# levia-than/neptune-pde-solver

Hardware: AMD Instinct MI355X
Metric: stencil-cell-updates/s (higher is better)
Workload: dtype f64

## Files before the change

### neptune-pde-solver_amd/csrc/kernels/apply_march2.hpp

```cpp
#pragma once
#include "apply_march.hpp"

namespace neptune_hip {

template <class T, int NIN>
struct March2Params {
  const T* in[NIN];
  T* out;
  int32_t N0, N1, N2;
  int32_t plb[3], pub[3];
  int64_t olb[3];
  int32_t rI0, rI1;
  int32_t chunk;
  uint32_t nJ, nK;
};

template <class T, class FP, int NS>
struct March2Geom {
  static constexpr int VK = 16 / (int)sizeof(T), G = 64 / (int)sizeof(T);
  static constexpr int R0 = FP::R0, R1 = FP::R1, R2 = FP::R2;
  static constexpr int HG = G / 2 > VK ? G / 2 : VK;
  static constexpr int MK = (NS * R2 + HG - 1) / HG * HG;
  static constexpr int SPAN = kWave * VK, KEEPK = SPAN - 2 * MK;
  static constexpr int MJ = NS * R1;
  static constexpr int WARM = 2 * R0 * (NS - 1);
};

template <class T, int NIN>
struct Leapfrog2Params : March2Params<T, NIN> {
  T* out_v;
};

template <class Body, class T, int NIN, class FP, int NS, int RJ, int WJ, int MINW, bool LF = false>
__global__ __launch_bounds__(kWave* WJ, MINW) void neptune_apply_march2(
    std::conditional_t<LF, Leapfrog2Params<T, NIN>, March2Params<T, NIN>> P, Body body) {
  using V = typename Vec16<T>::type;
  using GM = March2Geom<T, FP, NS>;
  constexpr int VK = GM::VK, R0 = GM::R0, R1 = GM::R1, R2 = GM::R2, NP = 2 * R0 + 1;
  static_assert(NS >= 2 && NS <= 3, "two or three applies per pass");
  static_assert(!LF || (NS == 2 && NIN >= 2), "leapfrog: two stages, input 1 = the previous state");
  constexpr int TJ = RJ * WJ;
  constexpr int MK = GM::MK, SPAN = GM::SPAN;
  static_assert(R0 >= 1 && R0 <= 2 && R1 >= 1 && R1 <= 2 && R2 >= 1 && R2 <= 2 && !FP::BOX && FP::HALO_MASK == 1u, "star of input 0, radius 1..2");
  static_assert(RJ >= R1 && R2 <= VK && TJ > 2 * GM::MJ, "window too small for the footprint");
  constexpr int NQ = (NS - 1) * R0 + 1;
  constexpr int NF = NIN > 1 ? NIN - 1 : 1;
  __shared__ V lds[2][WJ][NS][2 * R1][kWave];

  const int lane = threadIdx.x & (kWave - 1);
  const int w = __builtin_amdgcn_readfirstlane(threadIdx.x >> 6);
  const uint32_t vb = xcd_remap(blockIdx.x, gridDim.x);
  const uint32_t kt = vb % P.nK;
  const uint32_t t = vb / P.nK;
  const uint32_t jt = t % P.nJ;
  const uint32_t ct = t / P.nJ;

  const int32_t Jb = (int32_t)(jt * (TJ - 2 * GM::MJ)) - GM::MJ;
  const int32_t j0 = Jb + w * RJ;
  const int32_t kw = (int32_t)(kt * GM::KEEPK) - MK;
  const int32_t k0 = kw + lane * VK;
  const int32_t kc = k0 < 0 ? 0 : (k0 > P.N2 - VK ? P.N2 - VK : k0);
  const uint32_t lane_b = (uint32_t)kc * (uint32_t)sizeof(T);
  uint32_t rowb[RJ];
  static_for<RJ>([&](auto rc) {
    constexpr int r = rc;
    int32_t j = j0 + r;
    j = j < 0 ? 0 : (j >= P.N1 ? P.N1 - 1 : j);
    rowb[r] = (uint32_t)j * (uint32_t)P.N2 * (uint32_t)sizeof(T);
  });
  const int64_t plane_b = (int64_t)P.N1 * P.N2 * (int64_t)sizeof(T);

  const int32_t ib = P.rI0 + (int32_t)ct * P.chunk;
  const int32_t ie = (ib + P.chunk < P.rI1) ? ib + P.chunk : P.rI1;
  if (ib >= ie) return;

  auto load_plane = [&](const T* field, int32_t ip, V(&rows)[RJ]) {
    const int32_t ic = ip < 0 ? 0 : (ip >= P.N0 ? P.N0 - 1 : ip);
    const char* base = reinterpret_cast<const char*>(field) + (int64_t)ic * plane_b;
    static_for<RJ>([&](auto rc) {
      constexpr int r = rc;
      rows[r] = *reinterpret_cast<const V*>(base + (rowb[r] + lane_b));
    });
  };

  bool row_keep[RJ], in_j[RJ], in_k[VK];
  static_for<RJ>([&](auto rc) {
    constexpr int r = rc;
    const int32_t j = j0 + r;
    row_keep[r] = j >= Jb + GM::MJ && j < Jb + TJ - GM::MJ && j >= 0 && j < P.N1;
    in_j[r] = j >= P.plb[1] && j < P.pub[1];
  });
  static_for<VK>([&](auto ec) {
    constexpr int e = ec;
    in_k[e] = (k0 + e) >= P.plb[2] && (k0 + e) < P.pub[2];
  });
  const bool lane_keep = k0 >= kw + MK && k0 < kw + SPAN - MK && k0 >= 0 && k0 < P.N2;

  auto stage = [&](const V(&pl)[NP][RJ], const V(&above)[R1], const V(&below)[R1], const V(&fx)[NF][NQ][RJ], const V(&xp)[RJ],
                   auto qc, int32_t ip, V(&res)[RJ]) {
    constexpr int q = decltype(qc)::value;
    V ring[1][NP][RJ + 2 * R1];
    T lft[1][1][RJ + 2 * R1][R2], rgt[1][1][RJ + 2 * R1][R2];
    V pt[NIN][RJ];
    static_for<RJ>([&](auto rc) {
      constexpr int r = rc;
      static_for<NP>([&](auto pc) { constexpr int pp = pc; ring[0][pp][r + R1] = pl[pp][r]; });
      static_for<R2>([&](auto xc) {
        constexpr int x = xc;
        constexpr int dl = R2 - x, dr = x + 1;
        lft[0][0][r + R1][x] = from_prev<true>(pl[R0][r][VK - dl], pl[R0][r][0], lane);
        rgt[0][0][r + R1][x] = from_next<true>(pl[R0][r][dr - 1], pl[R0][r][VK - 1], lane);
      });
      static_for<NIN>([&](auto nc) {
        constexpr int n = nc;
        if constexpr (LF && n == 1) pt[n][r] = xp[r];
        else if constexpr (n > 0) pt[n][r] = fx[n - 1][q][r];
      });
    });
    static_for<R1>([&](auto xc) {
      constexpr int x = xc;
      ring[0][R0][x] = above[x];
      ring[0][R0][RJ + R1 + x] = below[x];
    });
    const bool in_i = ip >= P.plb[0] && ip < P.pub[0];
    const int64_t li = (int64_t)ip + P.olb[0];
    static_for<RJ>([&](auto rc) {
      constexpr int r = rc;
      const int64_t lj = (int64_t)(j0 + r) + P.olb[1];
      static_for<VK>([&](auto ec) {
        constexpr int e = ec;
        const int64_t lk = (int64_t)(k0 + e) + P.olb[2];
        MarchAcc<T, 3, NIN, FP, RJ, r, e, false> acc{ring, lft, rgt, pt, li, lj, lk};
        const T val = body(acc);
        const T through = pl[R0][r][e];
        res[r][e] = (in_i && in_j[r] && in_k[e]) ? val : OutsideOf<Body, T>::apply(body, through);
      });
    });
  };

  V ring[NS][NP][RJ];
  V un[RJ];
  V fx[NF][NQ][RJ], fn[NF][RJ];
  V wres[RJ];
  const int32_t i0 = ib - GM::WARM;
  static_for<NP - 1>([&](auto pc) { constexpr int pp = pc; load_plane(P.in[0], i0 + NS * R0 - 2 * R0 + pp, ring[0][pp]); });
  load_plane(P.in[0], i0 + NS * R0, un);
  if constexpr (NIN > 1) {
    static_for<NIN - 1>([&](auto nc) {
      constexpr int n = nc;
      if constexpr (!(LF && n == 0))
        static_for<NQ - 1>([&](auto qc) { constexpr int q = qc; load_plane(P.in[n + 1], i0 + q, fx[n][q]); });
      load_plane(P.in[n + 1], i0 + NQ - 1, fn[n]);
    });
  }
  static_for<NS - 1>([&](auto kc) {
    constexpr int k = kc + 1;
    static_for<NP - 1>([&](auto pc) { constexpr int pp = pc; static_for<RJ>([&](auto rc) { constexpr int r = rc; ring[k][pp][r] = ring[0][0][r]; }); });
  });

  for (int32_t i = i0; i < ie; ++i) {
    static_for<RJ>([&](auto rc) { constexpr int r = rc; ring[0][NP - 1][r] = un[r]; });
    if constexpr (NIN > 1)
      static_for<NIN - 1>([&](auto nc) { constexpr int n = nc; static_for<RJ>([&](auto rc) { constexpr int r = rc; fx[n][NQ - 1][r] = fn[n][r]; }); });
    const int buf = (i - i0) & 1;
    static_for<NS>([&](auto kc) {
      constexpr int k = kc;
      static_for<R1>([&](auto xc) {
        constexpr int x = xc;
        lds[buf][w][k][x][lane] = ring[k][R0][x];
        lds[buf][w][k][R1 + x][lane] = ring[k][R0][RJ - R1 + x];
      });
    });
    __syncthreads();
    V above[NS][R1], below[NS][R1];
    static_for<NS>([&](auto kc) {
      constexpr int k = kc;
      static_for<R1>([&](auto xc) {
        constexpr int x = xc;
        above[k][x] = ring[k][R0][0];
        below[k][x] = ring[k][R0][RJ - 1];
        if (w > 0) above[k][x] = lds[buf][w - 1][k][R1 + x][lane];
        if (w < WJ - 1) below[k][x] = lds[buf][w + 1][k][x][lane];
      });
    });
    if (i + NS * R0 + 1 <= ie - 1 + NS * R0) {
      load_plane(P.in[0], i + NS * R0 + 1, un);
      if constexpr (NIN > 1) static_for<NIN - 1>([&](auto nc) { constexpr int n = nc; load_plane(P.in[n + 1], i + NQ, fn[n]); });
    }
    static_for<NS>([&](auto kc) {
      constexpr int k = kc;
      constexpr int q = (NS - k - 1) * R0;
      const V(&xp)[RJ] = (LF && k == 0) ? fx[0][NQ - 1] : ring[0][0];
      if constexpr (k + 1 < NS) stage(ring[k], above[k], below[k], fx, xp, std::integral_constant<int, q>{}, i + q, ring[k + 1][NP - 1]);
      else stage(ring[k], above[k], below[k], fx, xp, std::integral_constant<int, 0>{}, i, wres);
    });
    if (i >= ib && lane_keep) {
      char* obase = reinterpret_cast<char*>(P.out) + (int64_t)i * plane_b;
      static_for<RJ>([&](auto rc) {
        constexpr int r = rc;
        if (row_keep[r]) __builtin_nontemporal_store(wres[r], reinterpret_cast<V*>(obase + (rowb[r] + lane_b)));
      });
    }
    if constexpr (LF) {
      if (i + R0 >= ib && i + R0 < ie && lane_keep) {
        char* obase = reinterpret_cast<char*>(P.out_v) + (int64_t)(i + R0) * plane_b;
        static_for<RJ>([&](auto rc) {
          constexpr int r = rc;
          if (row_keep[r]) __builtin_nontemporal_store(ring[1][NP - 1][r], reinterpret_cast<V*>(obase + (rowb[r] + lane_b)));
        });
      }
    }
    static_for<NS>([&](auto kc) {
      constexpr int k = kc;
      static_for<NP - 1>([&](auto pc) { constexpr int pp = pc; static_for<RJ>([&](auto rc) { constexpr int r = rc; ring[k][pp][r] = ring[k][pp + 1][r]; }); });
    });
    if constexpr (NIN > 1)
      static_for<NIN - 1>([&](auto nc) {
        constexpr int n = nc;
        if constexpr (!(LF && n == 0))
          static_for<NQ - 1>([&](auto qc) { constexpr int q = qc; static_for<RJ>([&](auto rc) { constexpr int r = rc; fx[n][q][r] = fx[n][q + 1][r]; }); });
      });
  }
}


struct March2R2Params {
  const void* in[NEPTUNE_HIP_MAX_INPUTS];
  void* out;
  int32_t N0, N1;
  int32_t plb[2], pub[2];
  int64_t olb[2];
  int32_t rI0, rI1;
  int32_t chunk;
  uint32_t nK;
};

template <class FP>
constexpr bool march2_rank2_footprint() {
  return FP::MARCH_OK && !FP::BOX && FP::HALO_MASK == 1u && FP::R0 >= 1 && FP::R0 <= 2 && FP::R1 == 0 && FP::R2 >= 1 && FP::R2 <= 2;
}

struct Leapfrog2R2Params : March2R2Params {
  void* out_v;
};

template <class Body, class T, int NIN, class FP, int NS, int PF, bool LF = false>
__global__ __launch_bounds__(256) void neptune_apply_march2_rank2(std::conditional_t<LF, Leapfrog2R2Params, March2R2Params> P, Body body) {
  using V = typename Vec16<T>::type;
  using GM = March2Geom<T, FP, NS>;
  constexpr int VK = GM::VK, R0 = GM::R0, R2 = GM::R2, NP = 2 * R0 + 1, MK = GM::MK, SPAN = GM::SPAN, KEEPK = GM::KEEPK;
  static_assert(NS >= 2 && NS <= 3 && march2_rank2_footprint<FP>() && R2 <= VK, "window constants");
  static_assert(!LF || (NS == 2 && NIN >= 2), "leapfrog: two stages, input 1 = the previous state");
  constexpr int NQ = (NS - 1) * R0 + 1;
  constexpr int NF = NIN > 1 ? NIN - 1 : 1;
  const int lane = threadIdx.x & (kWave - 1);
  const uint32_t gw = blockIdx.x * (blockDim.x / kWave) + (threadIdx.x >> 6);
  const uint32_t kt = gw % P.nK, ct = gw / P.nK;
  const int32_t kw = (int32_t)(kt * KEEPK) - MK;
  const int32_t k0 = kw + lane * VK;
  const int32_t kc = k0 < 0 ? 0 : (k0 > P.N1 - VK ? P.N1 - VK : k0);
  const int32_t ib = P.rI0 + (int32_t)ct * P.chunk;
  const int32_t ie = (ib + P.chunk < P.rI1) ? ib + P.chunk : P.rI1;
  if (ib >= ie) return;
  T* out = static_cast<T*>(P.out);
  auto load_row = [&](int n, int32_t ip) -> V {
    const int32_t ic = ip < 0 ? 0 : (ip >= P.N0 ? P.N0 - 1 : ip);
    return *reinterpret_cast<const V*>(static_cast<const T*>(P.in[n]) + (int64_t)ic * P.N1 + kc);
  };
  bool in_k[VK];
  static_for<VK>([&](auto ec) { constexpr int e = ec; in_k[e] = (k0 + e) >= P.plb[1] && (k0 + e) < P.pub[1]; });
  const bool lane_keep = k0 >= kw + MK && k0 < kw + SPAN - MK && k0 >= 0 && k0 < P.N1;

  auto stage = [&](const V(&pl)[NP], const V(&fx)[NF][NQ], const V& xp, auto qc, int32_t ip) -> V {
    constexpr int q = decltype(qc)::value;
    V ring[1][NP][1];
    T lft[1][1][1][R2], rgt[1][1][1][R2];
    V pt[NIN][1];
    static_for<NP>([&](auto pc) { constexpr int pp = pc; ring[0][pp][0] = pl[pp]; });
    static_for<R2>([&](auto xc) {
      constexpr int x = xc;
      constexpr int dl = R2 - x, dr = x + 1;
      lft[0][0][0][x] = from_prev<true>(pl[R0][VK - dl], pl[R0][0], lane);
      rgt[0][0][0][x] = from_next<true>(pl[R0][dr - 1], pl[R0][VK - 1], lane);
    });
    static_for<NIN>([&](auto nc) {
      constexpr int n = nc;
      if constexpr (LF && n == 1) pt[n][0] = xp;
      else if constexpr (n > 0) pt[n][0] = fx[n - 1][q];
    });
    const bool in_i = ip >= P.plb[0] && ip < P.pub[0];
    const int64_t li = (int64_t)ip + P.olb[0];
    V res;
    static_for<VK>([&](auto ec) {
      constexpr int e = ec;
      const int64_t lk = (int64_t)(k0 + e) + P.olb[1];
      MarchAcc<T, 2, NIN, FP, 1, 0, e, false> acc{ring, lft, rgt, pt, li, 0, lk};
      const T val = body(acc);
      res[e] = (in_i && in_k[e]) ? val : OutsideOf<Body, T>::apply(body, pl[R0][e]);
    });
    return res;
  };

  V ring[NS][NP];
  V un[PF];
  V fx[NF][NQ], fn[NF][PF];
  const int32_t i0 = ib - GM::WARM;
  static_for<NP - 1>([&](auto pc) { constexpr int pp = pc; ring[0][pp] = load_row(0, i0 + NS * R0 - 2 * R0 + pp); });
  static_for<PF>([&](auto dc) { constexpr int d = dc; un[d] = load_row(0, i0 + NS * R0 + d); });
  if constexpr (NIN > 1) {
    static_for<NIN - 1>([&](auto nc) {
      constexpr int n = nc;
      if constexpr (!(LF && n == 0)) static_for<NQ - 1>([&](auto qc) { constexpr int q = qc; fx[n][q] = load_row(n + 1, i0 + q); });
      static_for<PF>([&](auto dc) { constexpr int d = dc; fn[n][d] = load_row(n + 1, i0 + NQ - 1 + d); });
    });
  }
  static_for<NS - 1>([&](auto kc2) { constexpr int k = kc2 + 1; static_for<NP - 1>([&](auto pc) { constexpr int pp = pc; ring[k][pp] = ring[0][0]; }); });
  auto step = [&](int32_t i, auto slot_c) {
    constexpr int slot = slot_c;
    ring[0][NP - 1] = un[slot];
    if constexpr (NIN > 1) static_for<NIN - 1>([&](auto nc) { constexpr int n = nc; fx[n][NQ - 1] = fn[n][slot]; });
    if (i + NS * R0 + PF <= ie - 1 + NS * R0) {
      un[slot] = load_row(0, i + NS * R0 + PF);
      if constexpr (NIN > 1) static_for<NIN - 1>([&](auto nc) { constexpr int n = nc; fn[n][slot] = load_row(n + 1, i + NQ - 1 + PF); });
    }
    V w;
    static_for<NS>([&](auto kc2) {
      constexpr int k = kc2;
      constexpr int q = (NS - k - 1) * R0;
      const V& xp = (LF && k == 0) ? fx[0][NQ - 1] : ring[0][0];
      if constexpr (k + 1 < NS) ring[k + 1][NP - 1] = stage(ring[k], fx, xp, std::integral_constant<int, q>{}, i + q);
      else w = stage(ring[k], fx, xp, std::integral_constant<int, 0>{}, i);
    });
    if (i >= ib && lane_keep) __builtin_nontemporal_store(w, reinterpret_cast<V*>(out + (int64_t)i * P.N1 + kc));
    if constexpr (LF) {
      if (i + R0 >= ib && i + R0 < ie && lane_keep)
        __builtin_nontemporal_store(ring[1][NP - 1], reinterpret_cast<V*>(static_cast<T*>(P.out_v) + (int64_t)(i + R0) * P.N1 + kc));
    }
    static_for<NS>([&](auto kc2) { constexpr int k = kc2; static_for<NP - 1>([&](auto pc) { constexpr int pp = pc; ring[k][pp] = ring[k][pp + 1]; }); });
    if constexpr (NIN > 1)
      static_for<NIN - 1>([&](auto nc) {
        constexpr int n = nc;
        if constexpr (!(LF && n == 0)) static_for<NQ - 1>([&](auto qc) { constexpr int q = qc; fx[n][q] = fx[n][q + 1]; });
      });
  };
  for (int32_t i = i0; i < ie; i += PF) {
    static_for<PF>([&](auto phc) {
      constexpr int ph = phc;
      if (i + ph < ie) step(i + ph, phc);
    });
  }
}


template <class T, int NIN, class FP>
inline bool march2_rank2_eligible(const neptune_hip_apply_geom_t* g, const void* const* in, const void* out) {
  constexpr int G = 64 / (int)sizeof(T);
  if (!g || g->rank != 2 || g->num_inputs != NIN) return false;
  if (!march2_rank2_footprint<FP>()) return false;
  int64_t n[2];
  const int r[2] = {FP::R0, FP::R2};
  for (int d = 0; d < 2; ++d) {
    n[d] = g->out_ub[d] - g->out_lb[d];
    for (int k = 0; k < NIN; ++k)
      if (g->in_lb[k][d] != g->out_lb[d] || g->in_ub[k][d] != g->out_ub[d]) return false;
    if (g->lb[d] < g->ub[d] && (g->lb[d] - r[d] < g->out_lb[d] || g->ub[d] + r[d] > g->out_ub[d])) return false;
  }
  if (g->region_lb[1] != 0 || g->region_ub[1] != n[1]) return false;
  if (n[1] % G != 0 || n[1] < 2 * G || n[0] < 1 || n[0] >= 0x7fffffffLL || n[1] >= 0x7fffffffLL) return false;
  if ((uintptr_t)out % 64 != 0) return false;
  for (int k = 0; k < NIN; ++k)
    if (!in[k] || (uintptr_t)in[k] % 64 != 0) return false;
  return true;
}

template <class Body, class T, int NIN, class FP, int NS, bool LF = false>
inline int launch_march2_rank2(const Body& body, const neptune_hip_apply_geom_t* g, const void* const* in, void* out, hipStream_t stream,
                               int chunk_req, void* out_v = nullptr) {
  if (!march2_rank2_eligible<T, NIN, FP>(g, in, out) || geom_bounds_empty(g)) return NEPTUNE_HIP_EUNSUPPORTED;
  constexpr int KEEPK = March2Geom<T, FP, NS>::KEEPK, PF = 4;
  std::conditional_t<LF, Leapfrog2R2Params, March2R2Params> P{};
  if constexpr (LF) P.out_v = out_v;
  for (int k = 0; k < NIN; ++k) P.in[k] = in[k];
  P.out = out;
  P.N0 = (int32_t)(g->out_ub[0] - g->out_lb[0]);
  P.N1 = (int32_t)(g->out_ub[1] - g->out_lb[1]);
  for (int d = 0; d < 2; ++d) {
    P.plb[d] = (int32_t)(g->lb[d] - g->out_lb[d]);
    P.pub[d] = (int32_t)(g->ub[d] - g->out_lb[d]);
    P.olb[d] = g->out_lb[d];
  }
  P.rI0 = (int32_t)g->region_lb[0];
  P.rI1 = (int32_t)g->region_ub[0];
  if (P.rI1 <= P.rI0) return NEPTUNE_HIP_OK;
  P.nK = (uint32_t)((P.N1 + KEEPK - 1) / KEEPK);
  const int64_t rows = P.rI1 - P.rI0;
  int64_t chunk = chunk_req > 0 ? chunk_req : 256;
  while (chunk_req <= 0 && chunk > 32 && (int64_t)P.nK * ((rows + chunk - 1) / chunk) < 8192) chunk /= 2;
  if (chunk > rows) chunk = rows;
  P.chunk = (int32_t)chunk;
  const int64_t waves = (int64_t)P.nK * ((rows + chunk - 1) / chunk);
  const int64_t blocks = (waves + 3) / 4;
  if (blocks <= 0 || blocks > 0x7fffffffLL) return NEPTUNE_HIP_EUNSUPPORTED;
  hipLaunchKernelGGL((neptune_apply_march2_rank2<Body, T, NIN, FP, NS, PF, LF>), dim3((uint32_t)blocks), dim3(256), 0, stream, P, body);
  NEPTUNE_HIP_CHECK(hipGetLastError());
  return NEPTUNE_HIP_OK;
}

template <class FP>
constexpr bool march2_footprint() {
  return FP::MARCH_OK && !FP::BOX && FP::HALO_MASK == 1u && FP::R0 >= 1 && FP::R0 <= 2 && FP::R1 >= 1 && FP::R1 <= 2 && FP::R2 >= 1 && FP::R2 <= 2;
}
template <class T, int NIN, class FP>
inline bool march2_eligible(const neptune_hip_apply_geom_t* g, const void* const* in, const void* out) {
  constexpr int G = 64 / (int)sizeof(T);
  if (!g || g->rank != 3 || g->num_inputs != NIN) return false;
  if (!march2_footprint<FP>()) return false;
  int64_t n[3];
  for (int d = 0; d < 3; ++d) {
    n[d] = g->out_ub[d] - g->out_lb[d];
    for (int k = 0; k < NIN; ++k)
      if (g->in_lb[k][d] != g->out_lb[d] || g->in_ub[k][d] != g->out_ub[d]) return false;
    if (d > 0 && (g->region_lb[d] != 0 || g->region_ub[d] != n[d])) return false;
  }
  if (n[2] % G != 0 || n[2] < 2 * G || n[1] < 8 || n[0] < 1) return false;
  if (n[1] * n[2] * (int64_t)sizeof(T) >= 0x7fffffffLL) return false;
  if ((uintptr_t)out % 64 != 0) return false;
  for (int k = 0; k < NIN; ++k)
    if (!in[k] || (uintptr_t)in[k] % 64 != 0) return false;
  const int r[3] = {FP::R0, FP::R1, FP::R2};
  for (int d = 0; d < 3; ++d)
    if (g->lb[d] < g->ub[d] && (g->lb[d] - r[d] < g->out_lb[d] || g->ub[d] + r[d] > g->out_ub[d])) return false;
  return true;
}

template <class Body, class T, int NIN, class FP, int NS, int RJ, int WJ, int MINW, bool LF = false>
inline int launch_march2_shape(const Body& body, const neptune_hip_apply_geom_t* g, const void* const* in, void* out, hipStream_t stream,
                               int chunk_req, void* out_v = nullptr) {
  using GM = March2Geom<T, FP, NS>;
  constexpr int KEEPJ = RJ * WJ - 2 * GM::MJ, KEEPK = GM::KEEPK;
  std::conditional_t<LF, Leapfrog2Params<T, NIN>, March2Params<T, NIN>> P{};
  if constexpr (LF) P.out_v = static_cast<T*>(out_v);
  for (int k = 0; k < NIN; ++k) P.in[k] = static_cast<const T*>(in[k]);
  P.out = static_cast<T*>(out);
  P.N0 = (int32_t)(g->out_ub[0] - g->out_lb[0]);
  P.N1 = (int32_t)(g->out_ub[1] - g->out_lb[1]);
  P.N2 = (int32_t)(g->out_ub[2] - g->out_lb[2]);
  for (int d = 0; d < 3; ++d) {
    P.plb[d] = (int32_t)(g->lb[d] - g->out_lb[d]);
    P.pub[d] = (int32_t)(g->ub[d] - g->out_lb[d]);
    P.olb[d] = g->out_lb[d];
  }
  P.rI0 = (int32_t)g->region_lb[0];
  P.rI1 = (int32_t)g->region_ub[0];
  if (P.rI1 <= P.rI0) return NEPTUNE_HIP_OK;
  P.nJ = (uint32_t)((P.N1 + KEEPJ - 1) / KEEPJ);
  P.nK = (uint32_t)((P.N2 + KEEPK - 1) / KEEPK);
  const int64_t planes = P.rI1 - P.rI0;
  int64_t chunk = chunk_req > 0 ? chunk_req : 128;
  while (chunk_req <= 0 && chunk > 16 && (int64_t)P.nJ * P.nK * ((planes + chunk - 1) / chunk) < 512) chunk /= 2;
  if (chunk > planes) chunk = planes;
  P.chunk = (int32_t)chunk;
  const int64_t blocks = (int64_t)P.nJ * P.nK * ((planes + chunk - 1) / chunk);
  if (blocks <= 0 || blocks > 0x7fffffffLL) return NEPTUNE_HIP_EUNSUPPORTED;
  hipLaunchKernelGGL((neptune_apply_march2<Body, T, NIN, FP, NS, RJ, WJ, MINW, LF>), dim3((uint32_t)blocks), dim3(kWave * WJ), 0, stream,
                     P, body);
  NEPTUNE_HIP_CHECK(hipGetLastError());
  return NEPTUNE_HIP_OK;
}

template <class Body, class T, int NIN, class FP, int NS>
inline int launch_march2(const Body& body, const neptune_hip_apply_geom_t* g, const void* const* in, void* out, hipStream_t stream,
                         int chunk_req) {
  if (!march2_eligible<T, NIN, FP>(g, in, out)) return NEPTUNE_HIP_EUNSUPPORTED;
  if (geom_bounds_empty(g)) return NEPTUNE_HIP_EUNSUPPORTED;
  static const int shape = [] { const char* e = getenv("NEPTUNE_HIP_MARCH2"); return e ? atoi(e) : 0; }();
  constexpr bool wide = FP::R0 > 1 || FP::R1 > 1 || FP::R2 > 1;
  if constexpr (wide) {
    if constexpr (NS != 2) {
      return NEPTUNE_HIP_EUNSUPPORTED;
    } else {
      switch (shape) {
        default:
        case 0: return launch_march2_shape<Body, T, NIN, FP, 2, 3, 8, 1>(body, g, in, out, stream, chunk_req);
        case 1: return launch_march2_shape<Body, T, NIN, FP, 2, 4, 8, 1>(body, g, in, out, stream, chunk_req);
      }
    }
  } else if constexpr (NS == 2) {
    switch (shape) {
      default:
      case 0: return launch_march2_shape<Body, T, NIN, FP, 2, 3, 16, 1>(body, g, in, out, stream, chunk_req);
#if NEPTUNE_HIP_FULL_VARIANTS
      case 1: return launch_march2_shape<Body, T, NIN, FP, 2, 7, 8, 1>(body, g, in, out, stream, chunk_req);
      case 2: return launch_march2_shape<Body, T, NIN, FP, 2, 4, 8, 1>(body, g, in, out, stream, chunk_req);
      case 3: return launch_march2_shape<Body, T, NIN, FP, 2, 2, 16, 1>(body, g, in, out, stream, chunk_req);
#endif
    }
  } else {
    switch (shape) {
      default:
      case 0: return launch_march2_shape<Body, T, NIN, FP, 3, 3, 12, 1>(body, g, in, out, stream, chunk_req);
#if NEPTUNE_HIP_FULL_VARIANTS
      case 1: return launch_march2_shape<Body, T, NIN, FP, 3, 2, 12, 1>(body, g, in, out, stream, chunk_req);
      case 2: return launch_march2_shape<Body, T, NIN, FP, 3, 4, 8, 1>(body, g, in, out, stream, chunk_req);
      case 3: return launch_march2_shape<Body, T, NIN, FP, 3, 5, 8, 1>(body, g, in, out, stream, chunk_req);
#endif
    }
  }
}

template <class Body, class T, int RANK, int NIN, class FP, int NS = 2>
inline int launch_apply_chain(const Body& body, const neptune_hip_apply_geom_t* g, const void* const* in, void* out,
                              hipStream_t stream, const neptune_hip_launch_cfg_t* cfg) {
  if constexpr (RANK == 3 && march2_footprint<FP>()) {
    if (!g || !in || !out) return NEPTUNE_HIP_EINVAL;
    for (int k = 0; k < NIN; ++k)
      if (!in[k]) return NEPTUNE_HIP_EINVAL;
    if (cfg && cfg->kernel == NEPTUNE_HIP_KERNEL_DIRECT) return NEPTUNE_HIP_EUNSUPPORTED;
    const int rc = geom_validate(g);
    if (rc != NEPTUNE_HIP_OK) return rc;
    return launch_march2<Body, T, NIN, FP, NS>(body, g, in, out, stream, cfg ? cfg->chunk : 0);
  } else if constexpr (RANK == 2 && march2_rank2_footprint<FP>()) {
    if (!g || !in || !out) return NEPTUNE_HIP_EINVAL;
    for (int k = 0; k < NIN; ++k)
      if (!in[k]) return NEPTUNE_HIP_EINVAL;
    if (cfg && cfg->kernel == NEPTUNE_HIP_KERNEL_DIRECT) return NEPTUNE_HIP_EUNSUPPORTED;
    const int rc = geom_validate(g);
    if (rc != NEPTUNE_HIP_OK) return rc;
    return launch_march2_rank2<Body, T, NIN, FP, NS>(body, g, in, out, stream, cfg ? cfg->chunk : 0);
  } else {
    return NEPTUNE_HIP_EUNSUPPORTED;
  }
}
template <class Body, class T, int RANK, int NIN, class FP>
inline int launch_apply_twice(const Body& body, const neptune_hip_apply_geom_t* g, const void* const* in, void* out,
                              hipStream_t stream, const neptune_hip_launch_cfg_t* cfg) {
  return launch_apply_chain<Body, T, RANK, NIN, FP, 2>(body, g, in, out, stream, cfg);
}
template <class Body, class T, int RANK, int NIN, class FP>
inline int launch_apply_thrice(const Body& body, const neptune_hip_apply_geom_t* g, const void* const* in, void* out,
                               hipStream_t stream, const neptune_hip_launch_cfg_t* cfg) {
  return launch_apply_chain<Body, T, RANK, NIN, FP, 3>(body, g, in, out, stream, cfg);
}

template <int RANK, int NIN, class FP>
constexpr bool leapfrog2_footprint() {
  if constexpr (RANK == 3) return march2_footprint<FP>() && NIN <= ((FP::R0 > 1 || FP::R1 > 1 || FP::R2 > 1) ? 2 : 3);
  else if constexpr (RANK == 2) return march2_rank2_footprint<FP>();
  else return false;
}
template <class T, int NIN>
inline bool leapfrog2_buffers_ok(const neptune_hip_apply_geom_t* g, const void* const* in, const void* out_v, const void* out_w) {
  if (!out_v || !out_w || (uintptr_t)out_v % 64 != 0) return false;
  const size_t bytes = geom_box_bytes(g->out_lb, g->out_ub, g->rank, sizeof(T));
  if (buffers_overlap(out_v, bytes, out_w, bytes)) return false;
  for (int k = 0; k < NIN; ++k)
    if (buffers_overlap(in[k], bytes, out_v, bytes) || buffers_overlap(in[k], bytes, out_w, bytes)) return false;
  return true;
}

template <class Body, class T, int RANK, int NIN, class FP>
inline int launch_apply_leapfrog2(const Body& body, const neptune_hip_apply_geom_t* g, const void* const* in, void* out_v, void* out_w,
                                  hipStream_t stream, const neptune_hip_launch_cfg_t* cfg) {
  static_assert(NIN >= 2, "a two-level scheme has the previous state as input 1");
  if constexpr (leapfrog2_footprint<RANK, NIN, FP>()) {
    if (!g || !in || !out_v || !out_w) return NEPTUNE_HIP_EINVAL;
    for (int k = 0; k < NIN; ++k)
      if (!in[k]) return NEPTUNE_HIP_EINVAL;
    if (cfg && (cfg->kernel == NEPTUNE_HIP_KERNEL_DIRECT || cfg->variant >= 0)) return NEPTUNE_HIP_EUNSUPPORTED;
    const int rc = geom_validate(g);
    if (rc != NEPTUNE_HIP_OK) return rc;
    if (g->num_inputs != NIN || !leapfrog2_buffers_ok<T, NIN>(g, in, out_v, out_w)) return NEPTUNE_HIP_EUNSUPPORTED;
    const int chunk = cfg ? cfg->chunk : 0;
    if constexpr (RANK == 3) {
      if (!march2_eligible<T, NIN, FP>(g, in, out_w) || geom_bounds_empty(g)) return NEPTUNE_HIP_EUNSUPPORTED;
      if constexpr (FP::R0 > 1 || FP::R1 > 1 || FP::R2 > 1)
        return launch_march2_shape<Body, T, NIN, FP, 2, 3, 8, 1, true>(body, g, in, out_w, stream, chunk, out_v);
      else if constexpr (NIN == 2)
        return launch_march2_shape<Body, T, NIN, FP, 2, 3, 12, 1, true>(body, g, in, out_w, stream, chunk, out_v);
      else
        return launch_march2_shape<Body, T, NIN, FP, 2, 4, 8, 1, true>(body, g, in, out_w, stream, chunk, out_v);
    } else {
      return launch_march2_rank2<Body, T, NIN, FP, 2, true>(body, g, in, out_w, stream, chunk, out_v);
    }
  } else {
    return NEPTUNE_HIP_EUNSUPPORTED;
  }
}

}
```

Measured before the change: 385.9 billion.

## Use buffer load/store intrinsics and optional multi-plane prefetch in march2 kernel

```diff
diff --git a/neptune-pde-solver_amd/csrc/kernels/apply_march2.hpp b/neptune-pde-solver_amd/csrc/kernels/apply_march2.hpp
--- a/neptune-pde-solver_amd/csrc/kernels/apply_march2.hpp
+++ b/neptune-pde-solver_amd/csrc/kernels/apply_march2.hpp
@@ -31,13 +31,14 @@
   T* out_v;
 };
 
-template <class Body, class T, int NIN, class FP, int NS, int RJ, int WJ, int MINW, bool LF = false>
+template <class Body, class T, int NIN, class FP, int NS, int RJ, int WJ, int MINW, bool LF = false, int PF = 1>
 __global__ __launch_bounds__(kWave* WJ, MINW) void neptune_apply_march2(
     std::conditional_t<LF, Leapfrog2Params<T, NIN>, March2Params<T, NIN>> P, Body body) {
   using V = typename Vec16<T>::type;
   using GM = March2Geom<T, FP, NS>;
   constexpr int VK = GM::VK, R0 = GM::R0, R1 = GM::R1, R2 = GM::R2, NP = 2 * R0 + 1;
   static_assert(NS >= 2 && NS <= 3, "two or three applies per pass");
+  static_assert(PF >= 1 && PF <= 3, "one to three planes in flight");
   static_assert(!LF || (NS == 2 && NIN >= 2), "leapfrog: two stages, input 1 = the previous state");
   constexpr int TJ = RJ * WJ;
   constexpr int MK = GM::MK, SPAN = GM::SPAN;
@@ -74,12 +75,28 @@
   const int32_t ie = (ib + P.chunk < P.rI1) ? ib + P.chunk : P.rI1;
   if (ib >= ie) return;
 
+  using U4 = unsigned int __attribute__((ext_vector_type(4)));
+  uint32_t offb[RJ];
+  static_for<RJ>([&](auto rc) { constexpr int r = rc; offb[r] = rowb[r] + lane_b; });
+  auto plane_desc = [&](const void* field, int32_t ip) {
+    char* base = const_cast<char*>(static_cast<const char*>(field)) + (int64_t)ip * plane_b;
+    return __builtin_amdgcn_make_buffer_rsrc(base, (short)0, (int)plane_b, 0x00020000);
+  };
   auto load_plane = [&](const T* field, int32_t ip, V(&rows)[RJ]) {
     const int32_t ic = ip < 0 ? 0 : (ip >= P.N0 ? P.N0 - 1 : ip);
-    const char* base = reinterpret_cast<const char*>(field) + (int64_t)ic * plane_b;
+    const auto rs = plane_desc(field, ic);
     static_for<RJ>([&](auto rc) {
       constexpr int r = rc;
-      rows[r] = *reinterpret_cast<const V*>(base + (rowb[r] + lane_b));
+      rows[r] = __builtin_bit_cast(V, __builtin_amdgcn_raw_buffer_load_b128(rs, (int)offb[r], 0, 0));
+    });
+  };
+  constexpr uint32_t kDropped = 0x80000000u;
+  auto store_plane = [&](T* field, int32_t ip, const V(&rows)[RJ], bool on, const uint32_t(&soff)[RJ]) {
+    const int32_t ic = ip < 0 ? 0 : (ip >= P.N0 ? P.N0 - 1 : ip);
+    const auto rs = plane_desc(field, ic);
+    static_for<RJ>([&](auto rc) {
+      constexpr int r = rc;
+      __builtin_amdgcn_raw_buffer_store_b128(__builtin_bit_cast(U4, rows[r]), rs, (int)(on ? soff[r] : kDropped), 0, 2 );
     });
   };
 
@@ -95,6 +112,8 @@
     in_k[e] = (k0 + e) >= P.plb[2] && (k0 + e) < P.pub[2];
   });
   const bool lane_keep = k0 >= kw + MK && k0 < kw + SPAN - MK && k0 >= 0 && k0 < P.N2;
+  uint32_t soff[RJ];
+  static_for<RJ>([&](auto rc) { constexpr int r = rc; soff[r] = (row_keep[r] && lane_keep) ? offb[r] : kDropped; });
 
   auto stage = [&](const V(&pl)[NP][RJ], const V(&above)[R1], const V(&below)[R1], const V(&fx)[NF][NQ][RJ], const V(&xp)[RJ],
                    auto qc, int32_t ip, V(&res)[RJ]) {
@@ -139,18 +158,18 @@
   };
 
   V ring[NS][NP][RJ];
-  V un[RJ];
-  V fx[NF][NQ][RJ], fn[NF][RJ];
+  V un[PF][RJ];
+  V fx[NF][NQ][RJ], fn[NF][PF][RJ];
   V wres[RJ];
   const int32_t i0 = ib - GM::WARM;
   static_for<NP - 1>([&](auto pc) { constexpr int pp = pc; load_plane(P.in[0], i0 + NS * R0 - 2 * R0 + pp, ring[0][pp]); });
-  load_plane(P.in[0], i0 + NS * R0, un);
+  static_for<PF>([&](auto dc) { constexpr int d = dc; load_plane(P.in[0], i0 + NS * R0 + d, un[d]); });
   if constexpr (NIN > 1) {
     static_for<NIN - 1>([&](auto nc) {
       constexpr int n = nc;
       if constexpr (!(LF && n == 0))
         static_for<NQ - 1>([&](auto qc) { constexpr int q = qc; load_plane(P.in[n + 1], i0 + q, fx[n][q]); });
-      load_plane(P.in[n + 1], i0 + NQ - 1, fn[n]);
+      static_for<PF>([&](auto dc) { constexpr int d = dc; load_plane(P.in[n + 1], i0 + NQ - 1 + d, fn[n][d]); });
     });
   }
   static_for<NS - 1>([&](auto kc) {
@@ -158,10 +177,11 @@
     static_for<NP - 1>([&](auto pc) { constexpr int pp = pc; static_for<RJ>([&](auto rc) { constexpr int r = rc; ring[k][pp][r] = ring[0][0][r]; }); });
   });
 
-  for (int32_t i = i0; i < ie; ++i) {
-    static_for<RJ>([&](auto rc) { constexpr int r = rc; ring[0][NP - 1][r] = un[r]; });
+  auto step = [&](int32_t i, auto slot_c) {
+    constexpr int slot = slot_c;
+    static_for<RJ>([&](auto rc) { constexpr int r = rc; ring[0][NP - 1][r] = un[slot][r]; });
     if constexpr (NIN > 1)
-      static_for<NIN - 1>([&](auto nc) { constexpr int n = nc; static_for<RJ>([&](auto rc) { constexpr int r = rc; fx[n][NQ - 1][r] = fn[n][r]; }); });
+      static_for<NIN - 1>([&](auto nc) { constexpr int n = nc; static_for<RJ>([&](auto rc) { constexpr int r = rc; fx[n][NQ - 1][r] = fn[n][slot][r]; }); });
     const int buf = (i - i0) & 1;
     static_for<NS>([&](auto kc) {
       constexpr int k = kc;
@@ -183,9 +203,10 @@
         if (w < WJ - 1) below[k][x] = lds[buf][w + 1][k][x][lane];
       });
     });
-    if (i + NS * R0 + 1 <= ie - 1 + NS * R0) {
-      load_plane(P.in[0], i + NS * R0 + 1, un);
-      if constexpr (NIN > 1) static_for<NIN - 1>([&](auto nc) { constexpr int n = nc; load_plane(P.in[n + 1], i + NQ, fn[n]); });
+    {
+      const int32_t ahead = i + PF <= ie - 1 ? i + PF : ie - 1;
+      load_plane(P.in[0], ahead + NS * R0, un[slot]);
+      if constexpr (NIN > 1) static_for<NIN - 1>([&](auto nc) { constexpr int n = nc; load_plane(P.in[n + 1], ahead + NQ - 1, fn[n][slot]); });
     }
     static_for<NS>([&](auto kc) {
       constexpr int k = kc;
@@ -194,21 +215,9 @@
       if constexpr (k + 1 < NS) stage(ring[k], above[k], below[k], fx, xp, std::integral_constant<int, q>{}, i + q, ring[k + 1][NP - 1]);
       else stage(ring[k], above[k], below[k], fx, xp, std::integral_constant<int, 0>{}, i, wres);
     });
-    if (i >= ib && lane_keep) {
-      char* obase = reinterpret_cast<char*>(P.out) + (int64_t)i * plane_b;
-      static_for<RJ>([&](auto rc) {
-        constexpr int r = rc;
-        if (row_keep[r]) __builtin_nontemporal_store(wres[r], reinterpret_cast<V*>(obase + (rowb[r] + lane_b)));
-      });
-    }
+    store_plane(P.out, i, wres, i >= ib, soff);
     if constexpr (LF) {
-      if (i + R0 >= ib && i + R0 < ie && lane_keep) {
-        char* obase = reinterpret_cast<char*>(P.out_v) + (int64_t)(i + R0) * plane_b;
-        static_for<RJ>([&](auto rc) {
-          constexpr int r = rc;
-          if (row_keep[r]) __builtin_nontemporal_store(ring[1][NP - 1][r], reinterpret_cast<V*>(obase + (rowb[r] + lane_b)));
-        });
-      }
+      store_plane(P.out_v, i + R0, ring[1][NP - 1], i + R0 >= ib && i + R0 < ie, soff);
     }
     static_for<NS>([&](auto kc) {
       constexpr int k = kc;
@@ -220,7 +229,14 @@
         if constexpr (!(LF && n == 0))
           static_for<NQ - 1>([&](auto qc) { constexpr int q = qc; static_for<RJ>([&](auto rc) { constexpr int r = rc; fx[n][q][r] = fx[n][q + 1][r]; }); });
       });
-  }
+  };
+  __builtin_amdgcn_s_waitcnt(0x0f70);
+  int32_t i = i0;
+  for (; i + PF <= ie; i += PF) static_for<PF>([&](auto phc) { constexpr int ph = phc; step(i + ph, phc); });
+  static_for<PF - 1>([&](auto phc) {
+    constexpr int ph = phc;
+    if (i + ph < ie) step(i + ph, phc);
+  });
 }
 
 
@@ -433,7 +449,7 @@
   return true;
 }
 
-template <class Body, class T, int NIN, class FP, int NS, int RJ, int WJ, int MINW, bool LF = false>
+template <class Body, class T, int NIN, class FP, int NS, int RJ, int WJ, int MINW, bool LF = false, int PF = 1>
 inline int launch_march2_shape(const Body& body, const neptune_hip_apply_geom_t* g, const void* const* in, void* out, hipStream_t stream,
                                int chunk_req, void* out_v = nullptr) {
   using GM = March2Geom<T, FP, NS>;
@@ -462,7 +478,7 @@
   P.chunk = (int32_t)chunk;
   const int64_t blocks = (int64_t)P.nJ * P.nK * ((planes + chunk - 1) / chunk);
   if (blocks <= 0 || blocks > 0x7fffffffLL) return NEPTUNE_HIP_EUNSUPPORTED;
-  hipLaunchKernelGGL((neptune_apply_march2<Body, T, NIN, FP, NS, RJ, WJ, MINW, LF>), dim3((uint32_t)blocks), dim3(kWave * WJ), 0, stream,
+  hipLaunchKernelGGL((neptune_apply_march2<Body, T, NIN, FP, NS, RJ, WJ, MINW, LF, PF>), dim3((uint32_t)blocks), dim3(kWave * WJ), 0, stream,
                      P, body);
   NEPTUNE_HIP_CHECK(hipGetLastError());
   return NEPTUNE_HIP_OK;
@@ -473,7 +489,8 @@
                          int chunk_req) {
   if (!march2_eligible<T, NIN, FP>(g, in, out)) return NEPTUNE_HIP_EUNSUPPORTED;
   if (geom_bounds_empty(g)) return NEPTUNE_HIP_EUNSUPPORTED;
-  static const int shape = [] { const char* e = getenv("NEPTUNE_HIP_MARCH2"); return e ? atoi(e) : 0; }();
+  static const int form = [] { const char* e = getenv("NEPTUNE_HIP_MARCH2"); return e ? atoi(e) : 0; }();
+  const int shape = form % 10, pf = form / 10;
   constexpr bool wide = FP::R0 > 1 || FP::R1 > 1 || FP::R2 > 1;
   if constexpr (wide) {
     if constexpr (NS != 2) {
@@ -492,7 +509,9 @@
 #if NEPTUNE_HIP_FULL_VARIANTS
       case 1: return launch_march2_shape<Body, T, NIN, FP, 2, 7, 8, 1>(body, g, in, out, stream, chunk_req);
       case 2: return launch_march2_shape<Body, T, NIN, FP, 2, 4, 8, 1>(body, g, in, out, stream, chunk_req);
-      case 3: return launch_march2_shape<Body, T, NIN, FP, 2, 2, 16, 1>(body, g, in, out, stream, chunk_req);
+      case 3:
+        if (pf == 2) return launch_march2_shape<Body, T, NIN, FP, 2, 2, 16, 1, false, 2>(body, g, in, out, stream, chunk_req);
+        return launch_march2_shape<Body, T, NIN, FP, 2, 2, 16, 1>(body, g, in, out, stream, chunk_req);
 #endif
     }
   } else {
@@ -500,7 +519,9 @@
       default:
       case 0: return launch_march2_shape<Body, T, NIN, FP, 3, 3, 12, 1>(body, g, in, out, stream, chunk_req);
 #if NEPTUNE_HIP_FULL_VARIANTS
-      case 1: return launch_march2_shape<Body, T, NIN, FP, 3, 2, 12, 1>(body, g, in, out, stream, chunk_req);
+      case 1:
+        if (pf == 2) return launch_march2_shape<Body, T, NIN, FP, 3, 2, 12, 1, false, 2>(body, g, in, out, stream, chunk_req);
+        return launch_march2_shape<Body, T, NIN, FP, 3, 2, 12, 1>(body, g, in, out, stream, chunk_req);
       case 2: return launch_march2_shape<Body, T, NIN, FP, 3, 4, 8, 1>(body, g, in, out, stream, chunk_req);
       case 3: return launch_march2_shape<Body, T, NIN, FP, 3, 5, 8, 1>(body, g, in, out, stream, chunk_req);
 #endif
```

Result: no change. 383.4 billion (-0.6%).
